# Ashish424/G.P.U-PathTracer

Measured on AMD Instinct MI355X. Metric: Mrays/sec, cornell_dragon 1920x1080 (+ achieved GB/s against the memory roofline), higher is better.
Workload: dtype f32; 1 GPU; cornell_dragon_800k (800032 tris) 1920x1080 depth 4 diff + reference 8-sphere room, 16 spp per step; kernel=auto, parallelism=1 GPU, closed_scene=True

## Files before the change

### g.p.u-pathtracer_amd/_abi.py

```python
import ctypes as C
import os

_HERE = os.path.dirname(os.path.abspath(__file__))
PTMI_PATH = os.environ.get("PT_LIBPTMI") or os.path.join(_HERE, "csrc", "libptmi.so")
PTHOST_PATH = os.path.join(_HERE, "host", "libpthost.so")


class Camera(C.Structure):
    _fields_ = [("pos", C.c_float * 3), ("front", C.c_float * 3), ("right", C.c_float * 3),
                ("up", C.c_float * 3), ("dist", C.c_float), ("aspect", C.c_float),
                ("fov", C.c_float), ("_pad", C.c_float)]


class Sphere(C.Structure):
    _fields_ = [("pos_rad", C.c_float * 4), ("emi", C.c_float * 3), ("col", C.c_float * 3),
                ("mat", C.c_int32)]


class Material(C.Structure):
    _fields_ = [("col", C.c_float * 3), ("emi", C.c_float * 3), ("mat", C.c_int32), ("phong_expo", C.c_float)]


class DenoiseParams(C.Structure):
    _fields_ = [("width", C.c_int32), ("height", C.c_int32), ("iterations", C.c_int32),
# ... 24 lines not shown
    _fields_ = [("max_leaf_size", C.c_int32), ("min_leaf_size", C.c_int32), ("max_depth", C.c_int32),
                ("n_bins", C.c_int32), ("sah_node_cost", C.c_float), ("sah_tri_cost", C.c_float),
                ("split_alpha", C.c_float), ("n_spatial_bins", C.c_int32), ("optimize_passes", C.c_int32)]


class BvhStats(C.Structure):
    _fields_ = [("n_inner", C.c_uint64), ("n_leaves", C.c_uint64), ("n_tri_refs", C.c_uint64),
                ("max_depth", C.c_uint32), ("sah_cost", C.c_float), ("build_ms", C.c_double),
                ("opt_cost_before", C.c_float), ("opt_cost_after", C.c_float)]


MAT_DIFF, MAT_METAL, MAT_SPEC, MAT_REFR = 0, 1, 2, 3
FLAG_METAL_LITERAL_W = 1 << 0
FLAG_WRITE_RGBA = 1 << 1
FLAG_FACE_FORWARD, FLAG_COSINE_DIFF, FLAG_GLASS_FIX, FLAG_RUSSIAN_ROULETTE, FLAG_MISS_KEEPS_PATH = 1 << 2, 1 << 3, 1 << 4, 1 << 5, 1 << 6
FLAG_RR_CPU_TRACER = 1 << 7
FLAG_NEE = 1 << 8
FLAGS_SMALLPT = FLAG_FACE_FORWARD | FLAG_COSINE_DIFF | FLAG_RUSSIAN_ROULETTE | FLAG_MISS_KEEPS_PATH
FLAGS_CPU_TRACER = FLAG_FACE_FORWARD | FLAG_COSINE_DIFF | FLAG_RR_CPU_TRACER | FLAG_MISS_KEEPS_PATH
KERNEL_AUTO, KERNEL_MEGA_BVH2, KERNEL_PERSISTENT, KERNEL_WAVEFRONT = 0, 1, 3, 5
OPT_KERNEL, OPT_COUNTERS, OPT_TIMING, OPT_BATCH, OPT_TOP_NODES, OPT_OCCUPANCY, OPT_LDS_STACK, OPT_WALK, OPT_LEAF_MAX, OPT_TRI_TEST, OPT_REFILL, OPT_VOTE_NODE, OPT_VOTE_REC, OPT_WAVE_BATCH, OPT_SPHERE_LDS, OPT_BUILD_ALGO, OPT_REBUILD, OPT_PRESPLIT, OPT_WAVE_BLOCKS, OPT_OVERLAP, OPT_OPTIMIZE, OPT_WAVE_SAMPLES = 1, 2, 3, 4, 5, 6, 7, 8, 9, 10, 11, 12, 13, 14, 15, 16, 17, 18, 19, 21, 24, 25
OPT_FIRST_WALK, OPT_PACKET_STACK, OPT_FUSE_STAGES, OPT_LAST_ANYHIT = 26, 27, 28, 29
OPT_ROOT_CULL = 30

_vp, _sz, _i, _u32 = C.c_void_p, C.c_size_t, C.c_int, C.c_uint32
PTMI_SYMBOLS = [
    ("pt_abi_version", _i, []),
    ("pt_device_count", _i, []),
    ("pt_create", _i, [_i, C.POINTER(_vp)]),
    ("pt_destroy", _i, [_vp]),
    ("pt_last_error", C.c_char_p, [_vp]),
    ("pt_set_stream", _i, [_vp, _vp]),
    ("pt_set_option", _i, [_vp, _i, _i]),
    ("pt_sync", _i, [_vp]),
    ("pt_malloc", _i, [_vp, _sz, C.POINTER(_vp)]),
    ("pt_free", _i, [_vp, _vp]),
    ("pt_memset", _i, [_vp, _vp, _i, _sz]),
    ("pt_download", _i, [_vp, _vp, _vp, _sz]),
    ("pt_upload", _i, [_vp, _vp, _vp, _sz]),
    ("pt_upload_bvh", _i, [_vp, _vp, _sz, _vp, _sz, _vp, _sz]),
    ("pt_upload_spheres", _i, [_vp, C.POINTER(Sphere), _sz]),
    ("pt_render", _i, [_vp, _vp, _vp, C.POINTER(Camera), C.POINTER(Params), _u32]),
    ("pt_render_moments", _i, [_vp, _vp, _vp, _vp, C.POINTER(Camera), C.POINTER(Params), _u32]),
    ("pt_frame_error", _i, [_vp, _vp, C.c_int32, C.c_int32, C.c_uint64, C.c_float, C.POINTER(C.c_double), C.POINTER(C.c_uint64)]),
    ("pt_trace_rays", _i, [_vp, _vp, _sz, _i, _vp, _vp, _vp]),
    ("pt_render_aux", _i, [_vp, C.POINTER(Camera), C.POINTER(Params), _vp, _vp, _vp, _vp]),
# ... 80 lines not shown
```

### g.p.u-pathtracer_amd/csrc/pt_ctx.h

```cpp
#pragma once
#include <hip/hip_runtime.h>

#include <algorithm>
#include <climits>
#include <cstdint>
#include <string>
#include <type_traits>
#include <vector>

#include "../../include/ptmi.h"
#include "pt_kernels.h"

#ifndef PT_FIRST_WALK_DEFAULT
#define PT_FIRST_WALK_DEFAULT 1
#endif

struct TreeState {
    float4* d_nodes = nullptr;
    float4* d_tris = nullptr;
    bool records_woop = false;
    bool has_bvh = false;
    uint64_t wide_root = 0;
    uint64_t n_wide = 0, n_inner = 0, n_refs = 0, n_leaves = 0, scene_bytes = 0;
    uint32_t wide_top_layout = 0, wide_depth = 0;
// ... 35 lines not shown
    int opt_presplit = 0;
    int opt_optimize = 0;
    int opt_rebuild = 0;
    int opt_build_algo = 1;
    int opt_sph_lds = 1;
    int opt_vote_node = 1, opt_vote_rec = 1;
    int opt_refill = 8;
    int opt_top = 64;
    int opt_occ = 6;
    int opt_lstk = 16;
    int opt_walk = 2;
    int opt_leaf_max = 2;
    int opt_tri_test = 0;
    void* d_wave = nullptr;
    size_t wave_bytes = 0;
    int opt_wave_batch = 16;
    int opt_wave_samples = 16;
    int opt_wave_blocks = 8;
    int opt_first_walk = PT_FIRST_WALK_DEFAULT;
    int opt_packet_stack = PT_PACKET_STACK_MAX;
    int opt_fuse_stages = 1;
    int opt_last_anyhit = 1;
    int opt_root_cull = 1;
    struct AutoPick {
        static constexpr int TRIALS = 4, PENDING = 4, DECIDED = 5;
        uint64_t key = 0;
        int phase = 0;
        int choice = PT_KERNEL_PERSISTENT;
        hipEvent_t e[2 * TRIALS] = {nullptr, nullptr, nullptr, nullptr, nullptr, nullptr, nullptr, nullptr};
        float ms[2] = {0.f, 0.f};
        uint64_t used = 0;
    };
    static constexpr int N_PICKS = 8;
    AutoPick picks[N_PICKS];
    int pick_last = -1;
    uint64_t pick_tick = 0;
    uint64_t scene_gen = 0;
    uint64_t geom_gen = 0;
    hipEvent_t geom_ev = nullptr;
    struct Refit {
        uint64_t scene_gen = 0;
        const float4* items = nullptr;
        void* d_mem = nullptr;
        int4* bin_list = nullptr;
        int4* wide_list = nullptr;
        float* bin_box = nullptr;
// ... 121 lines not shown
```

### g.p.u-pathtracer_amd/csrc/pt_k_wave.hip

```cpp
#include "pt_ctx.h"

__device__ __forceinline__ int wf_block_rank(bool keep, int& total, int* s_cnt) {
    const unsigned long long m = __ballot(keep);
    const int w = threadIdx.x >> 6;
    const int in_wave = (int)__builtin_amdgcn_mbcnt_hi((uint32_t)(m >> 32), __builtin_amdgcn_mbcnt_lo((uint32_t)m, 0u));
    if ((threadIdx.x & 63) == 0) s_cnt[w] = __popcll(m);
    __syncthreads();
    int base = 0, tot = 0;
#pragma unroll
    for (int k = 0; k < PT_BLOCK / 64; k++) {
        const int c = s_cnt[k];
        if (k < w) base += c;
        tot += c;
    }
    total = tot;
    return base + in_wave;
}

__device__ __forceinline__ void wf_sphere_table() {
    if (threadIdx.x < 11 * PT_KSPHERES) {
        PT_KARGS(K);
        const float v = ((const __attribute__((address_space(4))) float*)&K.ksph[0])[threadIdx.x];
        ((float*)s_dyn)[threadIdx.x] = v;
        if (threadIdx.x % 11 < 4) ((float*)s_dyn)[88 + 4 * (threadIdx.x / 11) + threadIdx.x % 11] = v;
    }
    __syncthreads();
}

__global__ void __launch_bounds__(256) k_wf_prepare(const KParams P) {
    for (uint32_t i = threadIdx.x; i < P.spp; i += 256) P.wf.hashes[i] = pt_wang64(P.frame + i);
    for (uint32_t i = threadIdx.x; i < P.wf.queues_words; i += 256) P.wf.queues_all[i] = 0u;
}

__device__ __forceinline__ bool wf_slot_pixel(const KParams& P, uint32_t slot, uint32_t& s_idx, int& px, int& py) {
    if (slot >= P.wf.n_slots) return false;
    return pt_slot_pixel(P, slot, s_idx, px, py);
}

__device__ __forceinline__ float wf_anyhit_start(float ts) {
    return ts < PT_F32_MAX ? __uint_as_float(__float_as_uint(ts) + 1u) : ts;
}

template <bool COUNT, int OCC, int LSTK, bool FIRST, bool ANY = false>
__global__ void __launch_bounds__(PT_BLOCK, OCC) k_wf_extend(const KParams P) {
    const int tid = threadIdx.x;
    const int lane = tid & 63;
    TravOverflow<LSTK> stk_ovf;
    TravStack<LSTK, PT_BLOCK> stk(__builtin_amdgcn_readfirstlane(tid & ~63), stk_ovf);
    const bool cull = P.cull != 0;
    const uint32_t n_regions = (uint32_t)P.wf.n_regions;
    const uint32_t shard_regions = (n_regions + PT_SHARDS - 1) / PT_SHARDS;
    const int batch = P.batch;

    uint32_t next = 0, end = 0;
    bool empty = false;
    int shard = (int)(blockIdx.x & (PT_SHARDS - 1));

    bool live = false;
    uint32_t idx = 0;
    v3 o = V3(0.f, 0.f, 0.f), d = V3(0.f, 0.f, 0.f);
    TravState ts;
    ts.idx = ts.idy = ts.idz = ts.oodx = ts.oody = ts.oodz = 0.f;
    ts.node = PT_SENTINEL; ts.leaf = 0; ts.sp = 0;
    ts.h = pt_no_hit();
    TravCount tc;
    uint32_t n_rays = 0, it_begin = 0, act_begin = 0, it_loop = 0;

    for (;;) {
        if (COUNT) it_loop++;
        const unsigned long long idle = __ballot(!live);
        const int n_idle = __popcll(idle);
        if (!empty && (n_idle >= batch || n_idle == 64)) {
            const uint32_t rank = __builtin_amdgcn_mbcnt_hi((uint32_t)(idle >> 32), __builtin_amdgcn_mbcnt_lo((uint32_t)idle, 0u));
            uint32_t served = 0;
            for (int round = 0; round < 8 && served < (uint32_t)n_idle; round++) {
                if (next == end) {
                    bool got = false;
                    for (int tries = 0; tries < PT_SHARDS && !got; tries++) {
                        uint32_t k = 0;
                        if (lane == 0) k = atomicAdd(P.wf.queue + shard * PT_SHARD_STRIDE, 1u);
                        k = (uint32_t)__builtin_amdgcn_readfirstlane((int)k);
                        const uint32_t r = k * PT_SHARDS + (uint32_t)shard;
                        if (k < shard_regions && r < n_regions) {
                            next = r * PT_REGION;
                            if (FIRST) end = min(next + (uint32_t)PT_REGION, P.wf.n_slots);
                            else end = next + (uint32_t)__builtin_amdgcn_readfirstlane(P.wf.walk_in[r]);
                            got = true;
                        } else {
                            shard = (shard + 1) & (PT_SHARDS - 1);
                        }
                    }
                    if (!got) { empty = true; break; }
                }
                const uint32_t take = min((uint32_t)n_idle - served, end - next);
                if (!live && rank >= served && rank < served + take) {
                    idx = next + (rank - served);
                    float bound = PT_F32_MAX;
                    if (FIRST) {
                        uint32_t s_idx = 0;
                        int px = 0, py = 0;
                        if (wf_slot_pixel(P, idx, s_idx, px, py)) {
                            PathState ps;
                            path_begin_hashed(P, px, py, (uint64_t)((uint32_t)py * (uint32_t)P.W + (uint32_t)px), P.wf.hashes[s_idx], ps);
                            o = ps.o;
                            d = ps.d;
                            live = true;
                        }
                    } else {
                        const float4 a = pt_sld4(P.wf.ray0_in + idx), b = pt_sld4(P.wf.ray1_in + idx);
                        if (ANY) bound = pt_sld1((const float*)(P.wf.hit + idx));
                        o = V3(a.x, a.y, a.z);
                        d = V3(a.w, b.x, b.y);
                        live = true;
                    }
                    if (live) trav_begin(ts, o, d, stk, P.sc.wide_root);
                    if (ANY) ts.h.t = wf_anyhit_start(bound);
                }
                next += take;
                served += take;
            }
            if (COUNT && served) { it_begin++; act_begin += served; }
        }
        const unsigned long long busy = __ballot(live);
        if (!busy) {
            if (empty) break;
            continue;
        }
        const int n_dead = empty ? 64 - __popcll(busy) : 0;
        if (live) {
            const bool fin = trav_run_wide<COUNT, true, false, true, ANY>(ts, P.sc, o, d, cull, stk, tc, n_dead, batch);
            if (fin) {
                if (ANY) { if (ts.h.t == 0.0f) pt_sst1((float*)(P.wf.hit + idx), 0.0f); }
                else pt_sst2(P.wf.hit + idx, make_float2(ts.h.t, __int_as_float(ts.h.rec)));
                live = false;
                if (COUNT) n_rays++;
            }
        }
    }

// ... 78 lines not shown
    const v3 e = done ? col : ps.accu;
    if (FIRST) {
        pt_sst3(smp, V3(0.f + e.x, 0.f + e.y, 0.f + e.z));
    } else wf_add_emission(smp, e);
    return !done;
}

template <int LP>
__device__ __forceinline__ void wf_fold_region(const KParams& P, uint32_t region) {
    if (threadIdx.x >= 64) return;
    uint32_t s_idx = 0;
    int px = 0, py = 0;
    const bool in = wf_slot_pixel(P, region * PT_REGION + (threadIdx.x / LP) * (4u * LP), s_idx, px, py);
    pt_fold_pixel_grouped<LP>(P, in, in ? (size_t)py * (size_t)P.W + (size_t)px : 0, (int)(threadIdx.x % LP));
}

__device__ __forceinline__ float2 wf_sphere_bound(const KParams& P, const PathState& ps) {
    const SceneHit sh = pt_closest_sphere(P, ps.o, ps.d, pt_no_hit(), 0);
    return make_float2(sh.t, __int_as_float(sh.sph_id));
}

template <bool BOUND>
__device__ __forceinline__ int wf_survivor_slot(const KParams& P, bool alive, const PathState& ps, float ts, bool& walk_free, int& n_walk,
                                                int& total, int* s_cnt, int* s_cnt_free) {
    walk_free = false;
    if (P.wf.root_cull) {
        const WideNode root = wide_node_load_uniform(P.sc, P.sc.wide_root);
        if (alive) {
            TravState s;
            trav_ray(s, ps.o, ps.d);
            uint32_t key[4];
            wide_node_keys_raw(root, s.idx, s.idy, s.idz, s.oodx, s.oody, s.oodz, BOUND ? wf_anyhit_start(ts) : PT_F32_MAX, key);
            walk_free = (key[0] & key[1] & key[2] & key[3]) == 0xffffffffu;
        }
    }
    const int r = PT_SURVIVOR_RANK(P, alive && !walk_free, ps, n_walk, s_cnt);
    total = n_walk;
    if (!P.wf.root_cull) return r;
    int n_free;
    const int rf = PT_SURVIVOR_RANK(P, walk_free, ps, n_free, s_cnt_free);
    total += n_free;
    return walk_free ? n_walk + rf : r;
}

template <bool COUNT>
__device__ __forceinline__ void wf_region_counts(const KParams& P, uint32_t region, int n_walk, int total) {
    if (threadIdx.x != 0) return;
    P.wf.cnt_out[region] = total;
    P.wf.walk_out[region] = n_walk;
    if (COUNT && total != n_walk) {
        atomicAdd(&P.counters[PT_CNT_RAYS], (unsigned long long)(total - n_walk));
        atomicAdd(&P.counters[PT_CNT_WALK_FREE], (unsigned long long)(total - n_walk));
    }
}

template <bool COUNT, bool NEE, bool FIRST, bool LAST = false, int FOLD = 0, bool BOUND = false>
// ... 15 lines not shown
    bool have = (int)threadIdx.x < n_in;
    bool alive = false, tri_hit = false;
    PathState ps;
    NeeReq req;
    req.want = false;
    uint32_t pix = 0, s_idx = 0;
    int px = 0, py = 0;
    if (FIRST) have = wf_slot_pixel(P, (uint32_t)i, s_idx, px, py);
    if (have) {
        if (FIRST) {
            pix = (uint32_t)py * (uint32_t)P.W + (uint32_t)px;
            path_begin_hashed(P, px, py, (uint64_t)pix, P.wf.hashes[s_idx], ps);
        } else {
            const float4 a = pt_sld4(P.wf.ray0_in + i), b = pt_sld4(P.wf.ray1_in + i);
            ps.o = V3(a.x, a.y, a.z);
            ps.d = V3(a.w, b.x, b.y);
            pix = __float_as_uint(b.z);
            ps.nee_mask = 0;
            uint32_t sn = __float_as_uint(b.w);
            if (NEE) {
                ps.nee_mask = (pix >> PT_REC_PIXEL_BITS) | ((sn >> PT_REC_LIGHT_BIT) << 8);
                pix &= (1u << PT_REC_PIXEL_BITS) - 1u;
                sn &= (1u << PT_REC_LIGHT_BIT) - 1u;
            }
            s_idx = sn >> PT_REC_DRAW_BITS;
            ps.mask = V3(pt_sld1(P.wf.mask_in + i), pt_sld1(P.wf.mask_in + (size_t)P.wf.cap + i), pt_sld1(P.wf.mask_in + 2 * (size_t)P.wf.cap + i));
            ps.accu = V3(0.f, 0.f, 0.f);
            ps.depth = P.wf.bounce;
            ps.rng = pt_rng_init(P.wf.hashes[s_idx], (uint64_t)pix);
            ps.rng.n = sn & (PT_REC_MAX_DRAWS - 1u);
        }
        const float2 hh = pt_sld2(P.wf.hit + i);
        Hit h;
        h.t = hh.x;
        h.rec = __float_as_int(hh.y);
        h.tri = -1;
        tri_hit = h.t < PT_F32_MAX;
        if (tri_hit) {
            h.tri = 0;
            if (P.tri_matid) h.tri = __float_as_int(P.sc.nodes[h.rec].w);
        }
        alive = wf_shade_segment<NEE, FIRST, LAST>(P, ps, h, tri_hit, pt_sample_ptr(P, s_idx, (size_t)pix), &req);
    }
    float2 bound = make_float2(PT_F32_MAX, __int_as_float(-1));
    if (BOUND && alive) bound = wf_sphere_bound(P, ps);
    if (COUNT) {
        const uint32_t nh = wave_sum_u32(tri_hit ? 1u : 0u), np = wave_sum_u32(have && !alive ? 1u : 0u);
// ... 2 lines not shown
            atomicAdd(&P.counters[PT_CNT_PATHS], (unsigned long long)np);
        }
    }
    if (NEE) {
        int n_sh;
        const int rs = wf_block_rank(req.want, n_sh, s_cnt2);
        if (req.want) {
            const size_t j = (size_t)region * PT_REGION + (size_t)rs;
            P.wf.s_ray0[j] = make_float4(req.o.x, req.o.y, req.o.z, req.d.x);
            P.wf.s_ray1[j] = make_float4(req.d.y, req.d.z, __uint_as_float(pix), __uint_as_float(s_idx));
            P.wf.s_con[j] = make_float4(req.contrib.x, req.contrib.y, req.contrib.z, req.t_max);
        }
        if (threadIdx.x == 0) P.wf.s_cnt[region] = n_sh;
    }
    if (last) {
        if constexpr (FOLD > 0) {
            __syncthreads();
            wf_fold_region<FOLD>(P, region);
        }
        return;
    }
    int n_walk, total;
    bool walk_free;
    const int r = wf_survivor_slot<BOUND>(P, alive, ps, bound.x, walk_free, n_walk, total, s_cnt, s_cnt_free);
    if (alive) {
        const size_t j = (size_t)region * PT_REGION + (size_t)r;
        pt_sst4(P.wf.ray0_out + j, make_float4(ps.o.x, ps.o.y, ps.o.z, ps.d.x));
        pt_sst4(P.wf.ray1_out + j, make_float4(ps.d.y, ps.d.z, __uint_as_float(NEE ? (pix | ((ps.nee_mask & 0xffu) << PT_REC_PIXEL_BITS)) : pix),
                                              __uint_as_float((s_idx << PT_REC_DRAW_BITS) | ps.rng.n | (NEE ? (ps.nee_mask >> 8) << PT_REC_LIGHT_BIT : 0u))));
        pt_sst1(P.wf.mask_out + j, ps.mask.x);
        pt_sst1(P.wf.mask_out + (size_t)P.wf.cap + j, ps.mask.y);
        pt_sst1(P.wf.mask_out + 2 * (size_t)P.wf.cap + j, ps.mask.z);
        if (BOUND) pt_sst2(P.wf.hit + j, bound);
        else if (walk_free) pt_sst2(P.wf.hit + j, make_float2(pt_no_hit().t, __int_as_float(pt_no_hit().rec)));
    }
    wf_region_counts<COUNT>(P, region, n_walk, total);
}

template <bool COUNT, int FOLD>
__global__ void __launch_bounds__(PT_BLOCK) k_wf_shade_last_any(const KParams P) {
    const uint32_t region = blockIdx.x;
    const int n_in = P.wf.cnt_in[region];
    if (n_in == 0) {
        if constexpr (FOLD > 0) wf_fold_region<FOLD>(P, region);
        return;
    }
    wf_sphere_table();
    const size_t i = (size_t)region * PT_REGION + threadIdx.x;
    const bool have = (int)threadIdx.x < n_in;
    bool tri_hit = false;
    if (have) {
        const float4 b = pt_sld4(P.wf.ray1_in + i);
        const float2 hh = pt_sld2(P.wf.hit + i);
        const v3 mask = V3(pt_sld1(P.wf.mask_in + i), pt_sld1(P.wf.mask_in + (size_t)P.wf.cap + i), pt_sld1(P.wf.mask_in + 2 * (size_t)P.wf.cap + i));
        const uint32_t pix = __float_as_uint(b.z), s_idx = __float_as_uint(b.w) >> PT_REC_DRAW_BITS;
        float* smp = pt_sample_ptr(P, s_idx, (size_t)pix);
        const int sph = __float_as_int(hh.y);
        tri_hit = hh.x == 0.0f;
        if (!tri_hit && sph >= 0) {
            const float* t = (const float*)s_dyn + 11 * sph;
            wf_add_emission(smp, vadd(V3(0.f, 0.f, 0.f), vmul(mask, V3(t[4], t[5], t[6]))));
        } else if (!tri_hit) {
            wf_shade_miss<false>(smp, mask);
        }
    }
    if (COUNT) {
        const uint32_t nh = wave_sum_u32(tri_hit ? 1u : 0u), np = wave_sum_u32(have ? 1u : 0u);
        if ((threadIdx.x & 63) == 0) {
            atomicAdd(&P.counters[PT_CNT_HITS], (unsigned long long)nh);
            atomicAdd(&P.counters[PT_CNT_PATHS], (unsigned long long)np);
        }
    }
    if constexpr (FOLD > 0) {
        __syncthreads();
        wf_fold_region<FOLD>(P, region);
    }
}

// ... 4 lines not shown
    wf_sphere_table();
    const uint32_t region = blockIdx.x;
    const size_t i = (size_t)region * PT_REGION + threadIdx.x;
    uint32_t s_idx = 0;
    int px = 0, py = 0;
    const bool have = wf_slot_pixel(P, (uint32_t)i, s_idx, px, py);
    const uint32_t pix = (uint32_t)py * (uint32_t)P.W + (uint32_t)px;
    PathState ps;
    ps.o = ps.d = V3(0.f, 0.f, 0.f);
    if (have) path_begin_hashed(P, px, py, (uint64_t)pix, P.wf.hashes[s_idx], ps);
    TravCount tc;
    Hit h = trav_packet_wide<false>(P.sc, ps.o, ps.d, P.cull != 0, have, tc);
    bool alive = false;
    if (have) {
        const bool tri_hit = h.t < PT_F32_MAX;
        if (tri_hit && !P.tri_matid) h.tri = 0;
        alive = wf_shade_segment<false, true, false>(P, ps, h, tri_hit, pt_sample_ptr(P, s_idx, (size_t)pix), nullptr);
    }
    if (P.wf.bounce + 1 >= P.depth) return;
    float2 bound = make_float2(PT_F32_MAX, __int_as_float(-1));
    if (BOUND && alive) bound = wf_sphere_bound(P, ps);
    int n_walk, total;
    bool walk_free;
    const int r = wf_survivor_slot<BOUND>(P, alive, ps, bound.x, walk_free, n_walk, total, s_cnt, s_cnt_free);
    if (alive) {
        const size_t j = (size_t)region * PT_REGION + (size_t)r;
        pt_sst4(P.wf.ray0_out + j, make_float4(ps.o.x, ps.o.y, ps.o.z, ps.d.x));
        pt_sst4(P.wf.ray1_out + j, make_float4(ps.d.y, ps.d.z, __uint_as_float(pix), __uint_as_float((s_idx << PT_REC_DRAW_BITS) | ps.rng.n)));
        pt_sst1(P.wf.mask_out + j, ps.mask.x);
        pt_sst1(P.wf.mask_out + (size_t)P.wf.cap + j, ps.mask.y);
        pt_sst1(P.wf.mask_out + 2 * (size_t)P.wf.cap + j, ps.mask.z);
        if (BOUND) pt_sst2(P.wf.hit + j, bound);
        else if (walk_free) pt_sst2(P.wf.hit + j, make_float2(pt_no_hit().t, __int_as_float(pt_no_hit().rec)));
    }
    wf_region_counts<false>(P, region, n_walk, total);
}

__global__ void __launch_bounds__(PT_BLOCK) k_wf_resolve(const KParams P) {
    const int n_in = P.wf.s_cnt[blockIdx.x];
    if ((int)threadIdx.x >= n_in) return;
    const size_t i = (size_t)blockIdx.x * PT_REGION + threadIdx.x;
    const float4 c = P.wf.s_con[i];
    const float2 hh = P.wf.s_hit[i];
    if (hh.x < c.w) return;
    const float4 b = P.wf.s_ray1[i];
    const uint32_t pix = __float_as_uint(b.z), s_idx = __float_as_uint(b.w);
    float* smp = pt_sample_ptr(P, s_idx, (size_t)pix);
    smp[0] += c.x; smp[1] += c.y; smp[2] += c.z;
}

namespace ptmi {
// ... 68 lines not shown
    b.hit = (float2*)base;
    base += w.b_hit;
    b.cnt[0] = (int*)base;
    b.cnt[1] = (int*)(base + w.b_cnt);
    b.walk[0] = (int*)(base + 2 * w.b_cnt);
    b.walk[1] = (int*)(base + 3 * w.b_cnt);
    base += 4 * w.b_cnt;
    b.hashes = (unsigned long long*)base;
    base += w.b_hash;
    b.queues = (unsigned int*)base;
    b.nee = base + w.b_q;
    return b;
}

enum WaveExtend { EXT_CLOSEST, EXT_ANY, EXT_FIRST, EXT_PACKET, EXT_FUSED };
enum WaveShade { SHADE_PLAIN, SHADE_BOUND, SHADE_LAST, SHADE_LAST_ANY, SHADE_NONE };
struct WavePlan {
    bool count, nee, deep_stack;
    bool packet;
    bool fuse_first;
    int fold_lp;
    bool anyhit;
    bool root_cull;
    WaveExtend extend(uint32_t b, uint32_t depth) const {
        if (b == 0) return fuse_first ? EXT_FUSED : packet ? EXT_PACKET : EXT_FIRST;
        return anyhit && b + 1 == depth ? EXT_ANY : EXT_CLOSEST;
    }
    WaveShade shade(uint32_t b, uint32_t depth) const {
        if (b == 0 && fuse_first) return SHADE_NONE;
        if (anyhit && b + 1 >= depth) return SHADE_LAST_ANY;
        if (anyhit && b + 2 == depth) return SHADE_BOUND;
        if (b != 0 && !nee && !count && b + 1 >= depth) return SHADE_LAST;
        return SHADE_PLAIN;
    }
};
static WavePlan wave_plan(const pt_ctx* c, const KParams& P, const LaunchCfg& L, bool nee) {
    WavePlan p;
    p.count = L.count; p.nee = nee; p.deep_stack = L.lstk == 24;
    p.packet = c->opt_first_walk == 1 && 3 * c->tree.wide_depth + 2 <= (uint32_t)c->opt_packet_stack;
    const bool fuse = c->opt_fuse_stages != 0 && !nee && !L.count, tri_dark = P.tri_emi[0] == 0.f && P.tri_emi[1] == 0.f && P.tri_emi[2] == 0.f;
    p.fuse_first = fuse && p.packet;
    p.fold_lp = fuse && !L.moments && P.depth >= 2 && P.sgroup_log2 >= 2 && P.sgroup_log2 <= 4 && P.spp == (1u << P.sgroup_log2) ? (int)P.spp / 4 : 0;
    p.anyhit = (L.count ? c->opt_last_anyhit == 2 : c->opt_last_anyhit >= 1) && P.depth >= 2 && !nee && !P.tri_matid && tri_dark &&
               P.sc.n_spheres <= PT_KSPHERES && !c->tree.records_woop;
    p.root_cull = L.count ? c->opt_root_cull == 2 : c->opt_root_cull >= 1;
    return p;
}

constexpr size_t WF_LDS_SHADE = 15 * PT_KSPHERES * 4;
static hipError_t launch_extend(const WavePlan& p, WaveExtend kind, const KParams& Q, const LaunchCfg& L, int blocks_per_cu, hipStream_t s) {
    auto plain = [&](auto kernel, size_t n_blk, size_t lds) {
        hipLaunchKernelGGL(kernel, dim3((unsigned)n_blk), dim3(PT_BLOCK), lds, s, Q);
        return hipGetLastError();
    };
    const size_t n_reg = (size_t)Q.wf.n_regions;
    if (kind == EXT_FUSED)
        return p.anyhit && Q.depth == 2 ? plain(k_wf_extend_packet_shade<true>, n_reg, WF_LDS_SHADE) : plain(k_wf_extend_packet_shade<false>, n_reg, WF_LDS_SHADE);
    if (kind == EXT_PACKET) {
#ifdef PT_PACKET_RESIDENT_GRID
        const bool resident = true;
#else
        const bool resident = p.count;
#endif
        const size_t n_blk = resident ? std::min<size_t>(n_reg, (size_t)8 * L.n_cu) : n_reg;
        return p.count ? plain(k_wf_extend_packet<true>, n_blk, 0) : plain(k_wf_extend_packet<false>, n_blk, 0);
    }
    return with_bool(p.count, [&](auto count) {
        return with_bool(p.deep_stack, [&](auto deep) {
            constexpr int OCC = deep() ? 6 : 8, LSTK = deep() ? 24 : 16;
            auto go = [&](auto first, auto any) {
                return launch_resident(k_wf_extend<count(), OCC, LSTK, first(), any()>, (size_t)LSTK * PT_BLOCK * 4, blocks_per_cu, L.n_cu,
                                       (size_t)Q.wf.n_regions, s, Q);
            };
            if (kind == EXT_FIRST) return go(std::true_type{}, std::false_type{});
            if (kind == EXT_ANY) return go(std::false_type{}, std::true_type{});
            return go(std::false_type{}, std::false_type{});
        });
    });
}

static hipError_t launch_shade(const WavePlan& p, WaveShade kind, bool first, const KParams& Q, hipStream_t s) {
    auto go = [&](auto kernel) {
        hipLaunchKernelGGL(kernel, dim3((unsigned)Q.wf.n_regions), dim3(PT_BLOCK), WF_LDS_SHADE, s, Q);
        return hipGetLastError();
    };
    if (p.count) {
        if (kind == SHADE_LAST_ANY) return go(k_wf_shade_last_any<true, 0>);
        return with_bool(first, [&](auto f) {
            if (kind == SHADE_BOUND) return go(k_wf_shade<true, false, f(), false, 0, true>);
            return p.nee ? go(k_wf_shade<true, true, f()>) : go(k_wf_shade<true, false, f()>);
        });
    }
    if (kind == SHADE_LAST_ANY) return with_int<4, 2, 1, 0>(p.fold_lp, [&](auto lp) { return go(k_wf_shade_last_any<false, lp()>); });
    if (kind == SHADE_LAST) return with_int<4, 2, 1, 0>(p.fold_lp, [&](auto lp) { return go(k_wf_shade<false, false, false, true, lp()>); });
    return with_bool(first, [&](auto f) {
        if (kind == SHADE_BOUND) return go(k_wf_shade<false, false, f(), false, 0, true>);
        return p.nee ? go(k_wf_shade<false, true, f()>) : go(k_wf_shade<false, false, f()>);
    });
}

int render_wavefront(pt_ctx* c, KParams& P, const LaunchCfg& L, int work_tiles, bool& folded) {
    folded = false;
    WaveLayout w;
    int rc = wave_layout(c, P, work_tiles, w);
    if (rc == PT_OK) rc = wave_reserve(c, w);
    if (rc != PT_OK) return rc;
    const WaveBuffers buf = wave_carve((char*)c->d_wave, w);
    const WavePlan plan = wave_plan(c, P, L, w.nee);
    folded = plan.fold_lp != 0;
    P.wf.nee = w.nee ? 1 : 0;
    P.wf.root_cull = plan.root_cull ? 1 : 0;
    if (w.nee) {
        P.wf.s_ray0 = (float4*)buf.nee;
        P.wf.s_ray1 = (float4*)(buf.nee + w.b_ray);
        P.wf.s_con = (float4*)(buf.nee + 2 * w.b_ray);
        P.wf.s_hit = (float2*)(buf.nee + 3 * w.b_ray);
        P.wf.s_cnt = (int*)(buf.nee + 3 * w.b_ray + w.b_hit);
    }

    hipStream_t st = c->stream;
    P.sc.n_top = 0;
    P.sph_tab = 0;
    P.batch = c->opt_wave_batch;
    P.wf.hit = buf.hit;
    P.wf.hashes = buf.hashes;
    P.wf.queues_all = buf.queues;
    P.wf.queues_words = (uint32_t)w.q_words;
    P.wf.cap = (uint32_t)w.cap;
    P.wf.n_regions = (int)w.n_regions;
    P.wf.n_slots = (uint32_t)((size_t)work_tiles * 64);
    P.wf.bounce = 0;
    hipLaunchKernelGGL(k_wf_prepare, dim3(1), dim3(256), 0, st, P);
    HIP_TRY(c, hipGetLastError());
    if (stage_mark(c, PT_STAGE_GENERATE) != PT_OK) return PT_ERR_DEVICE;
// ... 29 lines not shown
```

### g.p.u-pathtracer_amd/csrc/pt_kernels.h

```cpp
#pragma once
#include "pt_math.h"
#include "../../include/ptmi.h"

#define PT_BLOCK 256
#define PT_BLOCK_RAYS 256
#define PT_TILE 8
#define PT_MAX_TOP 1024
#define PT_STACK_CAP 72
#define PT_SHARDS 8
#define PT_SHARD_STRIDE 32
#define PT_REGION 256

struct KScene {
    const float4* __restrict__ nodes;
    const float4* __restrict__ tris;
    const pt_sphere_d* __restrict__ spheres;
    int n_spheres;
    int has_bvh;
    int n_top;
    int stack_n;
    int top_base;
    int wide_root;
};

#define PT_KSPHERES 8

constexpr uint32_t PT_REC_DRAW_BITS = 12;
constexpr uint32_t PT_REC_LIGHT_BIT = 31;
constexpr uint32_t PT_REC_PIXEL_BITS = 24;
constexpr uint32_t PT_REC_MAX_DRAWS = 1u << PT_REC_DRAW_BITS, PT_REC_MAX_SAMPLES = 1u << (32 - PT_REC_DRAW_BITS),
                   PT_REC_MAX_SAMPLES_NEE = 1u << (PT_REC_LIGHT_BIT - PT_REC_DRAW_BITS);
struct KWave {
    const float4* __restrict__ ray0_in;
    const float4* __restrict__ ray1_in;
    const float* __restrict__ mask_in;
    float4* __restrict__ ray0_out;
    float4* __restrict__ ray1_out;
    float* __restrict__ mask_out;
    float2* __restrict__ hit;
    const int* __restrict__ walk_in;
    const int* __restrict__ cnt_in;
    int* __restrict__ cnt_out;
    int* __restrict__ walk_out;
    unsigned long long* hashes;
    unsigned int* queue;
    unsigned int* queues_all;
    uint32_t queues_words;
    uint32_t cap;
    int n_regions;
    uint32_t n_slots;
    float4* __restrict__ s_ray0;
    float4* __restrict__ s_ray1;
    float4* __restrict__ s_con;
    float2* __restrict__ s_hit;
    int* __restrict__ s_cnt;
    int nee;
    int root_cull;
    uint32_t bounce;
};

struct KParams {
    KScene sc;
    pt_sphere_d ksph[PT_KSPHERES];
    float* __restrict__ accum;
    uint32_t* __restrict__ rgba;
    unsigned long long* counters;
    pt_camera cam;
    int W, H;
    uint32_t depth;
    int cull;
    uint64_t frame, sample_index;
    uint32_t spp;
    int tri_mat;
    float tri_col[3], tri_emi[3], bk[3];
    float air_ior, glass_ior, phong;
    const int* tri_matid;
    const float4* mat_table;
    const float4* tri_lights;
    int n_tri_lights;
    uint32_t flags;
// ... 176 lines not shown
```

### g.p.u-pathtracer_amd/csrc/ptmi.hip

```cpp
#include <hip/hip_runtime.h>

#include <algorithm>
#include <cmath>
#include <cstdio>
#include <cstring>
#include <string>
#include <vector>

#include "pt_ctx.h"
#include "pt_scene_build.h"

static_assert(sizeof(pt_sphere) == 44, "pt_sphere must match the reference Sphere (44 B)");
static_assert(sizeof(pt_sphere_d) == sizeof(pt_sphere), "device sphere mirror");
static_assert(sizeof(pt_params) == 104 && sizeof(pt_camera) == 64 && sizeof(pt_counters) == 48, "ABI struct sizes (tests/test_host_and_abi.py)");

namespace ptmi {
thread_local std::string g_err;
}
using namespace ptmi;

namespace ptmi {
static int tree_cost_impl(pt_ctx* c, double* node_visits, double* tri_tests);

static bool auto_decide(pt_ctx* c, pt_ctx::AutoPick& a, bool wait) {
// ... 113 lines not shown
    {PT_OPT_OVERLAP, &pt_ctx::opt_overlap, OptionRow::FLAG, {}, PT_OK, ""},
    {PT_OPT_TOP_NODES, &pt_ctx::opt_top, OptionRow::RANGE, {0, PT_MAX_TOP}, PT_ERR_INVALID, "pt_set_option: top nodes must be 0..1024"},
    {PT_OPT_OCCUPANCY, &pt_ctx::opt_occ, OptionRow::SET, {4, 5, 6, 8}, PT_ERR_INVALID, "pt_set_option: occupancy must be 4, 5 (runs as 6), 6 or 8 waves per SIMD"},
    {PT_OPT_TRI_TEST, &pt_ctx::opt_tri_test, OptionRow::RANGE, {0, 1}, PT_ERR_INVALID, "pt_set_option: tri test must be 0 (Moller-Trumbore) or 1 (Woop)"},
    {PT_OPT_LEAF_MAX, &pt_ctx::opt_leaf_max, OptionRow::RANGE, {0, 1024}, PT_ERR_INVALID, "pt_set_option: leaf_max must be 0 (keep) .. 1024"},
    {PT_OPT_WALK, &pt_ctx::opt_walk, OptionRow::SET, {0, 1, 2, 4}, PT_ERR_INVALID, "pt_set_option: walk must be 0 (while-while), 1 (unified-step), 2 (wide) or 4 (wide, postponed leaf)"},
    {PT_OPT_REBUILD, &pt_ctx::opt_rebuild, OptionRow::RANGE, {0, 2}, PT_ERR_INVALID, "pt_set_option: rebuild must be 0 (keep the hierarchy), 1 (re-cluster) or 2 (keep the cheaper tree)"},
    {PT_OPT_PRESPLIT, &pt_ctx::opt_presplit, OptionRow::RANGE, {0, 100000}, PT_ERR_INVALID, "pt_set_option: presplit must be 0 (off) .. 100000 (per cent of diag/sqrt(n))"},
    {PT_OPT_BUILD_ALGO, &pt_ctx::opt_build_algo, OptionRow::RANGE, {0, 1}, PT_ERR_INVALID, "pt_set_option: build algorithm must be 0 (LBVH) or 1 (PLOC)"},
    {PT_OPT_WAVE_BATCH, &pt_ctx::opt_wave_batch, OptionRow::RANGE, {1, 64}, PT_ERR_INVALID, "pt_set_option: wave batch must be 1..64"},
    {PT_OPT_VOTE_NODE, &pt_ctx::opt_vote_node, OptionRow::RANGE, {1, 64}, PT_ERR_INVALID, "pt_set_option: vote weight must be 1..64"},
    {PT_OPT_VOTE_REC, &pt_ctx::opt_vote_rec, OptionRow::RANGE, {1, 64}, PT_ERR_INVALID, "pt_set_option: vote weight must be 1..64"},
    {PT_OPT_OPTIMIZE, &pt_ctx::opt_optimize, OptionRow::RANGE, {0, 16}, PT_ERR_INVALID, "pt_set_option: optimize passes must be 0 (off) .. 16"},
    {PT_OPT_WAVE_SAMPLES, &pt_ctx::opt_wave_samples, OptionRow::RANGE, {1, 64}, PT_ERR_INVALID, "pt_set_option: wave samples must be 1 (one sample of a tile per wave) .. 64"},
    {PT_OPT_WAVE_BLOCKS, &pt_ctx::opt_wave_blocks, OptionRow::RANGE, {1, 8}, PT_ERR_INVALID, "pt_set_option: wave blocks must be 1..8 per CU"},
    {PT_OPT_LDS_STACK, &pt_ctx::opt_lstk, OptionRow::SET, {0, 16, 24, 24}, PT_ERR_INVALID, "pt_set_option: LDS stack must be 0 (all 72 entries in LDS), 16 or 24 entries"},
    {PT_OPT_REFILL, &pt_ctx::opt_refill, OptionRow::RANGE, {1, 64}, PT_ERR_INVALID, "pt_set_option: refill must be 1..64"},
    {PT_OPT_BATCH, &pt_ctx::opt_batch, OptionRow::RANGE, {1, 64}, PT_ERR_INVALID, "pt_set_option: batch must be 1..64"},
    {PT_OPT_FIRST_WALK, &pt_ctx::opt_first_walk, OptionRow::RANGE, {0, 1}, PT_ERR_INVALID, "pt_set_option: first walk must be 0 (per lane) or 1 (wave-wide packets)"},
    {PT_OPT_PACKET_STACK, &pt_ctx::opt_packet_stack, OptionRow::RANGE, {2, PT_PACKET_STACK_MAX}, PT_ERR_INVALID, "pt_set_option: packet stack must be 2..72 entries"},
    {PT_OPT_FUSE_STAGES, &pt_ctx::opt_fuse_stages, OptionRow::RANGE, {0, 1}, PT_ERR_INVALID, "pt_set_option: fuse stages must be 0 (separate launches) or 1"},
    {PT_OPT_LAST_ANYHIT, &pt_ctx::opt_last_anyhit, OptionRow::RANGE, {0, 2}, PT_ERR_INVALID, "pt_set_option: last any-hit must be 0 (off), 1 (product launches) or 2 (instrumented launches too)"},
    {PT_OPT_ROOT_CULL, &pt_ctx::opt_root_cull, OptionRow::RANGE, {0, 2}, PT_ERR_INVALID, "pt_set_option: root cull must be 0 (off), 1 (product launches) or 2 (instrumented launches too)"},
};
}

extern "C" {

int pt_abi_version(void) { return PTMI_ABI_VERSION; }

int pt_device_count(void) {
    int n = 0;
    hipError_t e = hipGetDeviceCount(&n);
    if (e != hipSuccess) { g_err = std::string("hipGetDeviceCount: ") + hipGetErrorString(e); return PT_ERR_DEVICE; }
    return n;
}

const char* pt_last_error(const pt_ctx* ctx) { return ctx ? ctx->err.c_str() : g_err.c_str(); }

int pt_create(int device, pt_ctx** out) {
    if (!out) return fail(nullptr, PT_ERR_INVALID, "pt_create: out is null");
    *out = nullptr;
    int n = 0;
    hipError_t e = hipGetDeviceCount(&n);
    if (e != hipSuccess) return hip_fail(nullptr, e, "hipGetDeviceCount");
    if (device < 0 || device >= n) return fail(nullptr, PT_ERR_INVALID, "pt_create: no such device");
// ... 792 lines not shown
```

### include/ptmi.h

```cpp
#ifndef PTMI_H
#define PTMI_H

#include <stddef.h>
#include <stdint.h>

#ifdef __cplusplus
extern "C" {
#endif

#define PTMI_ABI_VERSION 3

typedef struct pt_ctx pt_ctx;

typedef enum pt_status {
    PT_OK = 0,
    PT_ERR_INVALID = -1,
    PT_ERR_DEVICE = -2,
    PT_ERR_NO_SCENE = -3,
    PT_ERR_NOMEM = -4,
    PT_ERR_UNSUPPORTED = -5
} pt_status;

enum { PT_MAT_DIFF = 0, PT_MAT_METAL = 1, PT_MAT_SPEC = 2, PT_MAT_REFR = 3 };

// ... 25 lines not shown
    PT_OPT_BATCH = 4,
    PT_OPT_TOP_NODES = 5,
    PT_OPT_OCCUPANCY = 6,
    PT_OPT_LDS_STACK = 7,
    PT_OPT_WALK = 8,
    PT_OPT_REFILL = 11,
    PT_OPT_VOTE_NODE = 12,
    PT_OPT_VOTE_REC = 13,
    PT_OPT_WAVE_BATCH = 14,
    PT_OPT_SPHERE_LDS = 15,
    PT_OPT_WAVE_BLOCKS = 19,
    PT_OPT_WAVE_SAMPLES = 25,
    PT_OPT_FIRST_WALK = 26,
    PT_OPT_PACKET_STACK = 27,
    PT_OPT_OVERLAP = 21,
    PT_OPT_BUILD_ALGO = 16,
    PT_OPT_REBUILD = 17,
    PT_OPT_OPTIMIZE = 24,
    PT_OPT_PRESPLIT = 18,
    PT_OPT_TRI_TEST = 10,
    PT_OPT_LEAF_MAX = 9,
    PT_OPT_FUSE_STAGES = 28,
    PT_OPT_LAST_ANYHIT = 29,
    PT_OPT_ROOT_CULL = 30
};

typedef struct pt_camera {
    float pos[3];
    float front[3];
    float right[3];
    float up[3];
    float dist;
    float aspect;
    float fov;
    float _pad;
} pt_camera;

typedef struct pt_sphere {
    float pos_rad[4];
    float emi[3];
    float col[3];
    int32_t mat;
} pt_sphere;

typedef struct pt_params {
    int32_t width, height;
    uint32_t depth;
// ... 107 lines not shown
```

Baseline: 17400 Mrays/s.

## Reuse shade-stage root-node test to seed wavefront extend traversal stack

The shade kernel already intersects surviving rays against the wide BVH root for culling. It now sorts the hit children and packs their order and count into spare high bits of the ray record. The extend kernel then pushes those children directly instead of re-testing the root node. This removes one wide-node load and slab test per ray per bounce, at the cost of reserving bits of the sample-index field (limiting spp) and extra masking when decoding.

```diff
diff --git a/g.p.u-pathtracer_amd/_abi.py b/g.p.u-pathtracer_amd/_abi.py
--- a/g.p.u-pathtracer_amd/_abi.py
+++ b/g.p.u-pathtracer_amd/_abi.py
@@ -70,6 +70,7 @@
 OPT_KERNEL, OPT_COUNTERS, OPT_TIMING, OPT_BATCH, OPT_TOP_NODES, OPT_OCCUPANCY, OPT_LDS_STACK, OPT_WALK, OPT_LEAF_MAX, OPT_TRI_TEST, OPT_REFILL, OPT_VOTE_NODE, OPT_VOTE_REC, OPT_WAVE_BATCH, OPT_SPHERE_LDS, OPT_BUILD_ALGO, OPT_REBUILD, OPT_PRESPLIT, OPT_WAVE_BLOCKS, OPT_OVERLAP, OPT_OPTIMIZE, OPT_WAVE_SAMPLES = 1, 2, 3, 4, 5, 6, 7, 8, 9, 10, 11, 12, 13, 14, 15, 16, 17, 18, 19, 21, 24, 25
 OPT_FIRST_WALK, OPT_PACKET_STACK, OPT_FUSE_STAGES, OPT_LAST_ANYHIT = 26, 27, 28, 29
 OPT_ROOT_CULL = 30
+OPT_ROOT_ENTRY = 33
 
 _vp, _sz, _i, _u32 = C.c_void_p, C.c_size_t, C.c_int, C.c_uint32
 PTMI_SYMBOLS = [
diff --git a/g.p.u-pathtracer_amd/csrc/pt_ctx.h b/g.p.u-pathtracer_amd/csrc/pt_ctx.h
--- a/g.p.u-pathtracer_amd/csrc/pt_ctx.h
+++ b/g.p.u-pathtracer_amd/csrc/pt_ctx.h
@@ -81,6 +81,7 @@
     int opt_fuse_stages = 1;
     int opt_last_anyhit = 1;
     int opt_root_cull = 1;
+    int opt_root_entry = 1;
     struct AutoPick {
         static constexpr int TRIALS = 4, PENDING = 4, DECIDED = 5;
         uint64_t key = 0;
diff --git a/g.p.u-pathtracer_amd/csrc/pt_k_wave.hip b/g.p.u-pathtracer_amd/csrc/pt_k_wave.hip
--- a/g.p.u-pathtracer_amd/csrc/pt_k_wave.hip
+++ b/g.p.u-pathtracer_amd/csrc/pt_k_wave.hip
@@ -41,8 +41,9 @@
     return ts < PT_F32_MAX ? __uint_as_float(__float_as_uint(ts) + 1u) : ts;
 }
 
-template <bool COUNT, int OCC, int LSTK, bool FIRST, bool ANY = false>
+template <bool COUNT, int OCC, int LSTK, bool FIRST, bool ANY = false, bool ENTRY = false>
 __global__ void __launch_bounds__(PT_BLOCK, OCC) k_wf_extend(const KParams P) {
+    static_assert(!(FIRST && ENTRY), "bounce 0's rays come from the camera: nobody ran their root step");
     const int tid = threadIdx.x;
     const int lane = tid & 63;
     TravOverflow<LSTK> stk_ovf;
@@ -65,6 +66,12 @@
     ts.h = pt_no_hit();
     TravCount tc;
     uint32_t n_rays = 0, it_begin = 0, act_begin = 0, it_loop = 0;
+    int root_l0 = 0, root_l1 = 0, root_l2 = 0, root_l3 = 0;
+    if (ENTRY) {
+        const float4 q2 = pt_uld4(P.sc.nodes, P.sc.wide_root + 2), q3 = pt_uld4(P.sc.nodes, P.sc.wide_root + 3);
+        root_l0 = __float_as_int(q2.z); root_l1 = __float_as_int(q2.w);
+        root_l2 = __float_as_int(q3.x); root_l3 = __float_as_int(q3.y);
+    }
 
     for (;;) {
         if (COUNT) it_loop++;
@@ -95,7 +102,7 @@
                 const uint32_t take = min((uint32_t)n_idle - served, end - next);
                 if (!live && rank >= served && rank < served + take) {
                     idx = next + (rank - served);
-                    float bound = PT_F32_MAX;
+                    float bound = PT_F32_MAX, b_w = 0.f;
                     if (FIRST) {
                         uint32_t s_idx = 0;
                         int px = 0, py = 0;
@@ -111,10 +118,23 @@
                         if (ANY) bound = pt_sld1((const float*)(P.wf.hit + idx));
                         o = V3(a.x, a.y, a.z);
                         d = V3(a.w, b.x, b.y);
+                        b_w = b.w;
                         live = true;
                     }
                     if (live) trav_begin(ts, o, d, stk, P.sc.wide_root);
                     if (ANY) ts.h.t = wf_anyhit_start(bound);
+                    if constexpr (ENTRY) {
+                        const uint32_t code = __float_as_uint(b_w) >> PT_REC_ENTRY_SHIFT, n = pt_entry_count(code);
+                        auto link = [&](uint32_t k) {
+                            const uint32_t c = pt_entry_child(code, k);
+                            return c == 0u ? root_l0 : (c == 1u ? root_l1 : (c == 2u ? root_l2 : root_l3));
+                        };
+                        if (n == 4u) { ts.sp++; stk.put(ts.sp, link(3)); }
+                        if (n >= 3u) { ts.sp++; stk.put(ts.sp, link(2)); }
+                        if (n >= 2u) { ts.sp++; stk.put(ts.sp, link(1)); }
+                        ts.node = link(0);
+                        if (COUNT && ts.node < 0) tc.leaves++;
+                    }
                 }
                 next += take;
                 served += take;
@@ -239,8 +259,9 @@
 
 template <bool BOUND>
 __device__ __forceinline__ int wf_survivor_slot(const KParams& P, bool alive, const PathState& ps, float ts, bool& walk_free, int& n_walk,
-                                                int& total, int* s_cnt, int* s_cnt_free) {
+                                                int& total, int* s_cnt, int* s_cnt_free, uint32_t& entry) {
     walk_free = false;
+    entry = 0u;
     if (P.wf.root_cull) {
         const WideNode root = wide_node_load_uniform(P.sc, P.sc.wide_root);
         if (alive) {
@@ -249,6 +270,11 @@
             uint32_t key[4];
             wide_node_keys_raw(root, s.idx, s.idy, s.idz, s.oodx, s.oody, s.oodz, BOUND ? wf_anyhit_start(ts) : PT_F32_MAX, key);
             walk_free = (key[0] & key[1] & key[2] & key[3]) == 0xffffffffu;
+            if (P.wf.root_entry && !walk_free) {
+                wide_sort4(key);
+                const uint32_t n = 1u + (key[1] != 0xffffffffu ? 1u : 0u) + (key[2] != 0xffffffffu ? 1u : 0u) + (key[3] != 0xffffffffu ? 1u : 0u);
+                entry = pt_entry_pack(n, key[0], key[1], key[2]) << PT_REC_ENTRY_SHIFT;
+            }
         }
     }
     const int r = PT_SURVIVOR_RANK(P, alive && !walk_free, ps, n_walk, s_cnt);
@@ -310,7 +336,7 @@
                 ps.nee_mask = (pix >> PT_REC_PIXEL_BITS) | ((sn >> PT_REC_LIGHT_BIT) << 8);
                 pix &= (1u << PT_REC_PIXEL_BITS) - 1u;
                 sn &= (1u << PT_REC_LIGHT_BIT) - 1u;
-            }
+            } else if (P.wf.root_entry) sn &= (1u << PT_REC_ENTRY_SHIFT) - 1u;
             s_idx = sn >> PT_REC_DRAW_BITS;
             ps.mask = V3(pt_sld1(P.wf.mask_in + i), pt_sld1(P.wf.mask_in + (size_t)P.wf.cap + i), pt_sld1(P.wf.mask_in + 2 * (size_t)P.wf.cap + i));
             ps.accu = V3(0.f, 0.f, 0.f);
@@ -359,12 +385,13 @@
     }
     int n_walk, total;
     bool walk_free;
-    const int r = wf_survivor_slot<BOUND>(P, alive, ps, bound.x, walk_free, n_walk, total, s_cnt, s_cnt_free);
+    uint32_t entry;
+    const int r = wf_survivor_slot<BOUND>(P, alive, ps, bound.x, walk_free, n_walk, total, s_cnt, s_cnt_free, entry);
     if (alive) {
         const size_t j = (size_t)region * PT_REGION + (size_t)r;
         pt_sst4(P.wf.ray0_out + j, make_float4(ps.o.x, ps.o.y, ps.o.z, ps.d.x));
         pt_sst4(P.wf.ray1_out + j, make_float4(ps.d.y, ps.d.z, __uint_as_float(NEE ? (pix | ((ps.nee_mask & 0xffu) << PT_REC_PIXEL_BITS)) : pix),
-                                              __uint_as_float((s_idx << PT_REC_DRAW_BITS) | ps.rng.n | (NEE ? (ps.nee_mask >> 8) << PT_REC_LIGHT_BIT : 0u))));
+                                              __uint_as_float((s_idx << PT_REC_DRAW_BITS) | ps.rng.n | (NEE ? (ps.nee_mask >> 8) << PT_REC_LIGHT_BIT : entry))));
         pt_sst1(P.wf.mask_out + j, ps.mask.x);
         pt_sst1(P.wf.mask_out + (size_t)P.wf.cap + j, ps.mask.y);
         pt_sst1(P.wf.mask_out + 2 * (size_t)P.wf.cap + j, ps.mask.z);
@@ -390,7 +417,8 @@
         const float4 b = pt_sld4(P.wf.ray1_in + i);
         const float2 hh = pt_sld2(P.wf.hit + i);
         const v3 mask = V3(pt_sld1(P.wf.mask_in + i), pt_sld1(P.wf.mask_in + (size_t)P.wf.cap + i), pt_sld1(P.wf.mask_in + 2 * (size_t)P.wf.cap + i));
-        const uint32_t pix = __float_as_uint(b.z), s_idx = __float_as_uint(b.w) >> PT_REC_DRAW_BITS;
+        const uint32_t pix = __float_as_uint(b.z);
+        const uint32_t s_idx = (__float_as_uint(b.w) & (P.wf.root_entry ? (1u << PT_REC_ENTRY_SHIFT) - 1u : ~0u)) >> PT_REC_DRAW_BITS;
         float* smp = pt_sample_ptr(P, s_idx, (size_t)pix);
         const int sph = __float_as_int(hh.y);
         tri_hit = hh.x == 0.0f;
@@ -441,11 +469,12 @@
     if (BOUND && alive) bound = wf_sphere_bound(P, ps);
     int n_walk, total;
     bool walk_free;
-    const int r = wf_survivor_slot<BOUND>(P, alive, ps, bound.x, walk_free, n_walk, total, s_cnt, s_cnt_free);
+    uint32_t entry;
+    const int r = wf_survivor_slot<BOUND>(P, alive, ps, bound.x, walk_free, n_walk, total, s_cnt, s_cnt_free, entry);
     if (alive) {
         const size_t j = (size_t)region * PT_REGION + (size_t)r;
         pt_sst4(P.wf.ray0_out + j, make_float4(ps.o.x, ps.o.y, ps.o.z, ps.d.x));
-        pt_sst4(P.wf.ray1_out + j, make_float4(ps.d.y, ps.d.z, __uint_as_float(pix), __uint_as_float((s_idx << PT_REC_DRAW_BITS) | ps.rng.n)));
+        pt_sst4(P.wf.ray1_out + j, make_float4(ps.d.y, ps.d.z, __uint_as_float(pix), __uint_as_float((s_idx << PT_REC_DRAW_BITS) | ps.rng.n | entry)));
         pt_sst1(P.wf.mask_out + j, ps.mask.x);
         pt_sst1(P.wf.mask_out + (size_t)P.wf.cap + j, ps.mask.y);
         pt_sst1(P.wf.mask_out + 2 * (size_t)P.wf.cap + j, ps.mask.z);
@@ -560,6 +589,7 @@
     int fold_lp;
     bool anyhit;
     bool root_cull;
+    bool root_entry;
     WaveExtend extend(uint32_t b, uint32_t depth) const {
         if (b == 0) return fuse_first ? EXT_FUSED : packet ? EXT_PACKET : EXT_FIRST;
         return anyhit && b + 1 == depth ? EXT_ANY : EXT_CLOSEST;
@@ -582,6 +612,7 @@
     p.anyhit = (L.count ? c->opt_last_anyhit == 2 : c->opt_last_anyhit >= 1) && P.depth >= 2 && !nee && !P.tri_matid && tri_dark &&
                P.sc.n_spheres <= PT_KSPHERES && !c->tree.records_woop;
     p.root_cull = L.count ? c->opt_root_cull == 2 : c->opt_root_cull >= 1;
+    p.root_entry = p.root_cull && !nee && P.spp < PT_REC_MAX_SAMPLES_ENTRY && (L.count ? c->opt_root_entry == 2 : c->opt_root_entry >= 1);
     return p;
 }
 
@@ -606,13 +637,15 @@
     return with_bool(p.count, [&](auto count) {
         return with_bool(p.deep_stack, [&](auto deep) {
             constexpr int OCC = deep() ? 6 : 8, LSTK = deep() ? 24 : 16;
-            auto go = [&](auto first, auto any) {
-                return launch_resident(k_wf_extend<count(), OCC, LSTK, first(), any()>, (size_t)LSTK * PT_BLOCK * 4, blocks_per_cu, L.n_cu,
+            auto go = [&](auto first, auto any, auto entry) {
+                return launch_resident(k_wf_extend<count(), OCC, LSTK, first(), any(), entry()>, (size_t)LSTK * PT_BLOCK * 4, blocks_per_cu, L.n_cu,
                                        (size_t)Q.wf.n_regions, s, Q);
             };
-            if (kind == EXT_FIRST) return go(std::true_type{}, std::false_type{});
-            if (kind == EXT_ANY) return go(std::false_type{}, std::true_type{});
-            return go(std::false_type{}, std::false_type{});
+            if (kind == EXT_FIRST) return go(std::true_type{}, std::false_type{}, std::false_type{});
+            return with_bool(p.root_entry, [&](auto entry) {
+                if (kind == EXT_ANY) return go(std::false_type{}, std::true_type{}, entry);
+                return go(std::false_type{}, std::false_type{}, entry);
+            });
         });
     });
 }
@@ -648,6 +681,7 @@
     folded = plan.fold_lp != 0;
     P.wf.nee = w.nee ? 1 : 0;
     P.wf.root_cull = plan.root_cull ? 1 : 0;
+    P.wf.root_entry = plan.root_entry ? 1 : 0;
     if (w.nee) {
         P.wf.s_ray0 = (float4*)buf.nee;
         P.wf.s_ray1 = (float4*)(buf.nee + w.b_ray);
diff --git a/g.p.u-pathtracer_amd/csrc/pt_kernels.h b/g.p.u-pathtracer_amd/csrc/pt_kernels.h
--- a/g.p.u-pathtracer_amd/csrc/pt_kernels.h
+++ b/g.p.u-pathtracer_amd/csrc/pt_kernels.h
@@ -30,6 +30,35 @@
 constexpr uint32_t PT_REC_PIXEL_BITS = 24;
 constexpr uint32_t PT_REC_MAX_DRAWS = 1u << PT_REC_DRAW_BITS, PT_REC_MAX_SAMPLES = 1u << (32 - PT_REC_DRAW_BITS),
                    PT_REC_MAX_SAMPLES_NEE = 1u << (PT_REC_LIGHT_BIT - PT_REC_DRAW_BITS);
+constexpr uint32_t PT_REC_ENTRY_BITS = 8, PT_REC_ENTRY_SHIFT = 32 - PT_REC_ENTRY_BITS;
+constexpr uint32_t PT_REC_MAX_SAMPLES_ENTRY = 1u << (PT_REC_ENTRY_SHIFT - PT_REC_DRAW_BITS);
+constexpr uint32_t pt_entry_pack(uint32_t n, uint32_t c0, uint32_t c1, uint32_t c2) {
+    return (c0 & 3u) | ((c1 & 3u) << 2) | ((c2 & 3u) << 4) | ((n - 1u) << 6);
+}
+constexpr uint32_t pt_entry_count(uint32_t code) { return (code >> 6) + 1u; }
+constexpr uint32_t pt_entry_child(uint32_t code, uint32_t k) {
+    return k < 3u ? (code >> (2u * k)) & 3u : (code ^ (code >> 2) ^ (code >> 4)) & 3u;
+}
+constexpr bool pt_entry_round_trips() {
+    uint32_t seen = 0;
+    for (uint32_t n = 1; n <= 4; n++)
+        for (uint32_t s = 0; s < 256; s++) {
+            const uint32_t c[4] = {s & 3u, (s >> 2) & 3u, (s >> 4) & 3u, (s >> 6) & 3u};
+            bool distinct = true;
+            for (uint32_t i = 0; i < n; i++)
+                for (uint32_t j = i + 1; j < n; j++) distinct = distinct && c[i] != c[j];
+            bool rest_zero = true;
+            for (uint32_t i = n; i < 4; i++) rest_zero = rest_zero && c[i] == 0u;
+            if (!distinct || !rest_zero) continue;
+            const uint32_t code = pt_entry_pack(n, c[0], c[1], c[2]);
+            if (code >= (1u << PT_REC_ENTRY_BITS) || pt_entry_count(code) != n) return false;
+            for (uint32_t k = 0; k < n; k++)
+                if (pt_entry_child(code, k) != c[k]) return false;
+            seen++;
+        }
+    return seen == 64u;
+}
+static_assert(pt_entry_round_trips(), "the entry code of PT_OPT_ROOT_ENTRY");
 struct KWave {
     const float4* __restrict__ ray0_in;
     const float4* __restrict__ ray1_in;
@@ -56,6 +85,7 @@
     int* __restrict__ s_cnt;
     int nee;
     int root_cull;
+    int root_entry;
     uint32_t bounce;
 };
 
diff --git a/g.p.u-pathtracer_amd/csrc/ptmi.hip b/g.p.u-pathtracer_amd/csrc/ptmi.hip
--- a/g.p.u-pathtracer_amd/csrc/ptmi.hip
+++ b/g.p.u-pathtracer_amd/csrc/ptmi.hip
@@ -159,6 +159,7 @@
     {PT_OPT_FUSE_STAGES, &pt_ctx::opt_fuse_stages, OptionRow::RANGE, {0, 1}, PT_ERR_INVALID, "pt_set_option: fuse stages must be 0 (separate launches) or 1"},
     {PT_OPT_LAST_ANYHIT, &pt_ctx::opt_last_anyhit, OptionRow::RANGE, {0, 2}, PT_ERR_INVALID, "pt_set_option: last any-hit must be 0 (off), 1 (product launches) or 2 (instrumented launches too)"},
     {PT_OPT_ROOT_CULL, &pt_ctx::opt_root_cull, OptionRow::RANGE, {0, 2}, PT_ERR_INVALID, "pt_set_option: root cull must be 0 (off), 1 (product launches) or 2 (instrumented launches too)"},
+    {PT_OPT_ROOT_ENTRY, &pt_ctx::opt_root_entry, OptionRow::RANGE, {0, 2}, PT_ERR_INVALID, "pt_set_option: root entry must be 0 (off), 1 (product launches) or 2 (instrumented launches too)"},
 };
 }
 
diff --git a/include/ptmi.h b/include/ptmi.h
--- a/include/ptmi.h
+++ b/include/ptmi.h
@@ -71,7 +71,8 @@
     PT_OPT_LEAF_MAX = 9,
     PT_OPT_FUSE_STAGES = 28,
     PT_OPT_LAST_ANYHIT = 29,
-    PT_OPT_ROOT_CULL = 30
+    PT_OPT_ROOT_CULL = 30,
+    PT_OPT_ROOT_ENTRY = 33
 };
 
 typedef struct pt_camera {
```

Measured after the change: 17640 Mrays/s, median of 6. 1.01x the previous value.
